# aletheia-labs/qp-zk-circuits-rm

Hardware: AMD Instinct MI355X
Metric: Wormhole proofs/sec (whole node) (higher is better)
Workload: dtype u64 (Goldilocks field); 1 GPU; batch256_wormhole_proofs_per_gpu; circuit=wormhole deg13 (135 wires), batch_per_gpu=256, provers_per_gpu=3, step_schedule=pipelined, parallelism=proofs sharded x1, RCCL gather of leaf proofs

## Files before the change

### include/qpgpu.h

```cpp
#ifndef QPGPU_H
#define QPGPU_H
#include <stddef.h>
#include <stdint.h>

#ifdef __cplusplus
extern "C" {
#endif

typedef enum {
    QP_OK = 0,
    QP_ERR_ARG = 1,
    QP_ERR_HIP = 2,
    QP_ERR_OOM = 3,
    QP_ERR_STATE = 4,
    QP_ERR_WITNESS = 5,
    QP_ERR_FORMAT = 6
} qp_status;

typedef struct qp_ctx qp_ctx;
typedef struct qp_batch qp_batch;

int qp_ctx_create(int device, qp_ctx **out);
void qp_ctx_destroy(qp_ctx *ctx);
const char *qp_ctx_last_error(const qp_ctx *ctx);
// ... 70 lines not shown
int qp_voting_circuit_new(int zero_knowledge, qp_circuit **out);
int qp_voting_commit(const qp_circuit *c, const qp_voting_inputs *in, qp_witness **out, char *err, size_t errcap);
int qp_aggregation_circuit_new(const uint8_t *inner_common, size_t len, uint32_t nproofs, qp_circuit **out);
typedef struct {
    const uint8_t *verifier_only;
    size_t vlen;
    const uint8_t *const *proofs;
    const size_t *lens;
    uint32_t nproofs;
    const uint64_t *zk_randomness;
} qp_aggregation_chunk;
int qp_aggregation_commit(const qp_circuit *c, const uint8_t *verifier_only, size_t vlen,
                          const uint8_t *const *proofs, const size_t *lens, uint32_t nproofs,
                          const uint64_t *zk_randomness, qp_witness **out, char *err, size_t errcap);
int qp_witness_wires(const qp_witness *w, uint64_t *out);
int qp_witness_public_inputs(const qp_witness *w, uint64_t *out, uint32_t cap, uint32_t *n);
void qp_witness_free(qp_witness *w);

typedef struct qp_prover qp_prover;
int qp_prover_new(qp_ctx *ctx, const qp_circuit *c, uint32_t max_batch, qp_prover **out);
void qp_prover_free(qp_prover *p);
int qp_prover_proof_size(const qp_prover *p, size_t *len);
int qp_prover_verifier_data(const qp_prover *p, uint8_t *out, size_t cap, size_t *len);
int qp_prover_prove(qp_prover *p, const qp_witness *const *w, uint32_t nproofs, uint8_t *out, size_t stride,
                    size_t *lens);
int qp_prover_prove_wires(qp_prover *p, const uint64_t *wires, const uint64_t *pis, uint32_t nproofs, uint8_t *out,
                          size_t stride, size_t *lens);
int qp_prover_prove_wormhole_inputs(qp_prover *p, const qp_wormhole_inputs *in, uint32_t nproofs, uint8_t *out,
                                    size_t stride, size_t *lens);
int qp_prover_prove_voting_inputs(qp_prover *p, const qp_voting_inputs *in, uint32_t nproofs, uint8_t *out,
                                  size_t stride, size_t *lens);
int qp_prover_prove_aggregation(qp_prover *p, const qp_aggregation_chunk *chunks, uint32_t nchunks, uint8_t *out,
                                size_t stride, size_t *lens);
int qp_prover_prove_wires_dev(qp_prover *p, const uint64_t *d_wires, const uint64_t *pis, uint32_t nproofs,
                              uint8_t *out, size_t stride, size_t *lens);
int qp_prover_set_timing(qp_prover *p, int enable);
int qp_prover_debug_force_pow(qp_prover *p, uint64_t witness, int enable);
int qp_prover_debug_drop_table(qp_prover *p, const char *name);
enum {
    QP_FOP_NT_ADD = 0,
    QP_FOP_NT_ADD4,
    QP_FOP_GFN_ADD,
    QP_FOP_GFN_ADD_C,
    QP_FOP_PF_ADD_C,
    QP_FOP_GL_ADD,
    QP_FOP_NT_SUB,
    QP_FOP_NT_SUB4,
    QP_FOP_GL_SUB,
    QP_FOP_NT_REDUCE,
    QP_FOP_GFN_REDUCE,
    QP_FOP_GL_REDUCE128,
    QP_FOP_PF_REDUCE_ROW,
    QP_FOP_PF_REDUCE_ROW_C,
    QP_FOP_PF_SUB_SMALL,
    QP_FOP_PF_MUL,
    QP_FOP_PF_MUL_C,
    QP_FOP_PF_MULK2,
    QP_FOP_PF_MULK3,
    QP_FOP_GL_MUL,
    QP_FOP_PF_SBOX,
    QP_FOP_PF_SBOX_C,
    QP_FOP_NT_MUL_POW2,
    QP_FOP_ACC3,
    QP_FOP_COUNT
};
int qp_debug_field_op(qp_ctx *ctx, uint32_t op, uint32_t param, const uint64_t *a, const uint64_t *b, uint64_t n,
                      uint64_t *out);
enum {
    QP_PFORM_PERMUTE_NC = 0,
    QP_PFORM_PERMUTE_CAPZ,
    QP_PFORM_ROUNDS1_L7,
    QP_PFORM_COOP_PERMUTE,
    QP_PFORM_ROW_PERMUTE,
    QP_PFORM_MDS_BLOCK,
    QP_PFORM_MDS_K,
    QP_PFORM_MDS_MADS,
    QP_PFORM_CAPZ_ROUND0,
    QP_PFORM_MDS_INIT_SPARSE,
    QP_PFORM_PARTIAL_GROUP,
    QP_PFORM_FULL_ROUND_DYN,
    QP_PFORM_PARTIAL_DYN,
    QP_PFORM_COOP_MDS,
    QP_PFORM_ROW_MDS,
    QP_PFORM_COUNT
};
int qp_debug_poseidon_op(qp_ctx *ctx, uint32_t form, uint32_t param, const uint64_t *states, uint64_t nstates,
                         uint64_t *out);
int qp_prover_set_host_threads(qp_prover *p, uint32_t nthreads);
int qp_prover_kernel_stats(qp_prover *p, double *ms, double *units, uint64_t *launches, uint32_t n, int reset);
int qp_prover_stage_times(qp_prover *p, double *ms, uint32_t n, int reset);

typedef struct qp_registry qp_registry;
int qp_registry_new(qp_ctx *ctx, const uint64_t *keys, uint64_t n, qp_registry **out);
void qp_registry_free(qp_registry *r);
int qp_registry_root(const qp_registry *r, uint64_t out[4]);
int qp_registry_size(const qp_registry *r, uint64_t *n, uint32_t *max_depth);
int qp_registry_paths(qp_registry *r, const uint64_t *idx, uint32_t nidx, uint64_t *siblings, uint32_t *path_bits,
                      uint32_t *depth);
int qp_registry_level(qp_registry *r, uint32_t level, uint64_t *out, uint64_t *len);
int qp_registry_build_times(const qp_registry *r, double ms[3]);

int qp_registry_new_commitments(qp_ctx *ctx, const uint64_t *leaves, uint64_t n, uint64_t capacity, qp_registry **out);
int qp_registry_append(qp_registry *r, const uint64_t *leaves, uint64_t k, uint64_t *first);
int qp_registry_replace(qp_registry *r, const uint64_t *idx, const uint64_t *leaves, uint32_t k);
int qp_registry_reserve(qp_registry *r, uint64_t new_capacity);
int qp_registry_state(const qp_registry *r, uint64_t *capacity, uint64_t *epoch);
typedef struct {
    uint64_t proposal_id[4];
    uint8_t vote;
    const uint64_t *zk_randomness;
} qp_vote_ballot;
int qp_prover_prove_voters(qp_prover *p, qp_registry *r, const uint64_t *idx, const qp_vote_ballot *ballots,
                           uint32_t nproofs, uint8_t *out, size_t stride, size_t *lens);

typedef enum {
    QP_BALLOT_COUNTED = 0,
    QP_BALLOT_PROOF_REJECTED = 1,
    QP_BALLOT_MALFORMED = 2,
    QP_BALLOT_WRONG_PROPOSAL = 3,
    QP_BALLOT_UNKNOWN_ROOT = 4,
    QP_BALLOT_BAD_VOTE = 5,
    QP_BALLOT_DOUBLE_VOTE = 6
} qp_ballot_status;
typedef struct qp_ballot_box qp_ballot_box;
struct qp_verifier;
typedef struct {
    uint32_t status;
    uint32_t verify_status;
    uint64_t number;
    uint64_t first;
} qp_ballot_result;
int qp_ballot_box_new(qp_ctx *ctx , const uint64_t proposal_id[4], const uint64_t *roots,
                      uint32_t nroots, uint64_t capacity, qp_ballot_box **out);
void qp_ballot_box_free(qp_ballot_box *b);
const char *qp_ballot_box_last_error(const qp_ballot_box *b);
int qp_ballot_box_accept_root(qp_ballot_box *b, const uint64_t root[4]);
int qp_ballot_box_cast(qp_ballot_box *b, struct qp_verifier *v, const uint8_t *const *proofs, const size_t *lens,
                       uint32_t n, qp_ballot_result *out);
int qp_ballot_box_cast_public(qp_ballot_box *b, const uint64_t *pis, const uint32_t *verdicts, uint32_t n,
                              qp_ballot_result *out);
int qp_ballot_box_reserve(qp_ballot_box *b, uint64_t new_capacity);
int qp_ballot_box_tally(const qp_ballot_box *b, uint64_t *yes, uint64_t *no);
int qp_ballot_box_state(const qp_ballot_box *b, uint64_t *cast, uint64_t *admitted, uint64_t *capacity);
int qp_ballot_box_entries(qp_ballot_box *b, uint64_t first, uint64_t k, uint64_t *nullifiers, uint64_t *numbers,
                          uint8_t *flags);
int qp_ballot_box_recount(qp_ballot_box *b, uint64_t out[4]);
int qp_ballot_box_cast_times(const qp_ballot_box *b, double ms[2]);


enum { QP_GATE_NOOP = 0 , QP_GATE_CONSTANT = 1 , QP_GATE_PUBLIC_INPUT = 2 ,
       QP_GATE_BASE_SUM = 3 , QP_GATE_ARITHMETIC = 4 , QP_GATE_POSEIDON = 5 ,
       QP_GATE_ARITHMETIC_EXTENSION = 6 , QP_GATE_MUL_EXTENSION = 7 ,
       QP_GATE_RANDOM_ACCESS = 8 , QP_GATE_EXPONENTIATION = 9 , QP_GATE_REDUCING = 10 ,
       QP_GATE_REDUCING_EXTENSION = 11 , QP_GATE_POSEIDON_MDS = 12 ,
       QP_GATE_COSET_INTERPOLATION = 13  };
#define QP_MAX_GATES 16

typedef struct {
    uint32_t num_gates;
    uint32_t kind[QP_MAX_GATES];
    uint32_t param[QP_MAX_GATES];
    uint32_t param2[QP_MAX_GATES];
    uint32_t param3[QP_MAX_GATES];
    uint32_t selector_index[QP_MAX_GATES];
    uint32_t num_selectors;
    uint32_t group_lo[QP_MAX_GATES], group_hi[QP_MAX_GATES];
// ... 72 lines not shown
```

### qp-zk-circuits-rm_amd/csrc/poseidon_fast.h

```cpp
#pragma once
#include <stdint.h>
#include <hip/hip_runtime.h>
#include "field_nc.h"
#include "poseidon.h"
#include "poseidon_partial_consts.h"

namespace pf {

using gfn::EPS;
using gfn::canon;
using gfn::hi32;
using gfn::lo32;
using gfn::mul;
using gfn::mul_c;

template <int C>
__device__ __forceinline__ uint64_t mad_c(uint32_t x, uint64_t add) {
  uint64_t r, cdummy;
  asm("v_mad_u64_u32 %0, %1, %2, %3, %4" : "=v"(r), "=s"(cdummy) : "v"(x), "i"(C), "v"(add));
  return r;
}
template <int C>
__device__ __forceinline__ uint64_t mad_cs(uint32_t x, uint64_t add) {
  uint64_t r, cdummy;
  asm("v_mad_u64_u32 %0, %1, %2, %3, %4" : "=v"(r), "=s"(cdummy) : "v"(x), "i"(C), "s"(add));
  return r;
}

__device__ __forceinline__ uint64_t reduce_row(uint64_t al, uint64_t ah) {
  uint64_t t, c1, c2;
  uint32_t e;
  asm("v_mad_u64_u32 %0, %1, %2, -1, %3" : "=v"(t), "=s"(c1) : "v"(hi32(ah)), "v"(al));
  uint32_t t0 = lo32(t), t1 = hi32(t);
  asm("v_add_co_u32_e64 %0, %1, %2, %3" : "=v"(t1), "=s"(c2) : "v"(t1), "v"(lo32(ah)));
  asm(QP_CWAIT "v_cndmask_b32_e64 %0, 0, -1, %1" : "=v"(e) : "s"(c2));
  const uint64_t tt = ((uint64_t)t1 << 32) | t0;
  uint64_t r;
  asm("v_mad_u64_u32 %0, %1, %2, 1, %3" : "=v"(r), "=s"(c1) : "v"(e), "v"(tt));
  return r;
}

__device__ __forceinline__ uint64_t reduce_row_c(uint64_t al, uint64_t ah) {
  const uint64_t t = al + (ah >> 32) * EPS;
  const uint32_t t1 = hi32(t) + lo32(ah);
  const uint64_t r = ((uint64_t)t1 << 32) | lo32(t);
  return t1 < lo32(ah) ? r + EPS : r;
}
__device__ __forceinline__ uint64_t sbox_c(uint64_t x) {
  const uint64_t x2 = mul_c(x, x);
  const uint64_t x3 = mul_c(x2, x);
  const uint64_t x4 = mul_c(x2, x2);
  return mul_c(x3, x4);
}

__device__ __forceinline__ uint64_t sbox(uint64_t x) {
  const uint64_t x2 = mul(x, x);
  const uint64_t x3 = mul(x2, x);
  const uint64_t x4 = mul(x2, x2);
  return mul(x3, x4);
}

__device__ __forceinline__ void sbox12(uint64_t s[12]) {
#pragma unroll
  for (int i = 0; i < 12; i++) s[i] = sbox(s[i]);
}

__device__ __forceinline__ uint64_t add_c(uint64_t a, uint64_t c) {
  const uint64_t s = a + c;
  return s + (s < c ? EPS : 0);
}

template <int R, int I>
__device__ __forceinline__ void row_terms(uint64_t &al, uint64_t &ah, const uint32_t lo[12], const uint32_t hi[12]) {
  if constexpr (I < 12) {
    constexpr int C = (int)ps::mds_circ(I) + ((R == 0 && I == 0) ? 8 : 0);
    al = mad_c<C>(lo[(I + R) % 12], al);
    ah = mad_c<C>(hi[(I + R) % 12], ah);
    row_terms<R, I + 1>(al, ah, lo, hi);
  }
}

template <int R>
__device__ __forceinline__ void mds_rows_k(uint64_t s[12], const uint32_t lo[12], const uint32_t hi[12],
                                           const uint64_t k[12]) {
  if constexpr (R < 12) {
    constexpr int C0 = (int)ps::mds_circ(0) + (R == 0 ? 8 : 0);
    uint64_t al = mad_cs<C0>(lo[R], k[R] & EPS);
// ... 199 lines not shown
    const uint32_t v = H ? hi32(s[J]) : lo32(s[J]);
    if constexpr (c != 0) asm("v_mad_u64_u32 %0, vcc, %1, %2, %0" : "+v"(S[K]) : "v"(v), "s"(c) : "vcc");
    if constexpr (K < 2) sparse_row0_h<T, J, H, K + 1>(S, s);
    else if constexpr (H == 0) sparse_row0_h<T, J, 1, 0>(S, s);
    else sparse_row0_h<T, J + 1, 0, 0>(S, s);
  }
}

__device__ __forceinline__ uint64_t sub_small(uint64_t r, uint32_t y0, uint32_t y1) {
  uint32_t r0 = lo32(r), r1 = hi32(r), e;
  uint64_t c;
  asm("v_sub_co_u32_e64 %0, %1, %2, %3" : "=v"(r0), "=s"(c) : "v"(r0), "v"(y0));
  asm(QP_CWAIT "v_subb_co_u32_e64 %0, %1, %2, %3, %4" : "=v"(r1), "=s"(c) : "v"(r1), "v"(y1), "s"(c));
  asm(QP_CWAIT "v_cndmask_b32_e64 %0, 0, -1, %1" : "=v"(e) : "s"(c));
  asm("v_sub_co_u32_e64 %0, %1, %2, %3" : "=v"(r0), "=s"(c) : "v"(r0), "v"(e));
  asm(QP_CWAIT "v_subb_co_u32_e64 %0, %1, %2, 0, %3" : "=v"(r1), "=s"(c) : "v"(r1), "s"(c));
  return ((uint64_t)r1 << 32) | r0;
}

constexpr int PF_GROUP = 4;
struct NoHook {
  __device__ __forceinline__ uint64_t operator()(int, uint64_t v) const { return v; }
};

template <int T0, int M, int L = 0>
__device__ __forceinline__ void group_gammas(uint64_t &al, uint64_t &ah, const uint32_t (*l)[3]) {
  if constexpr (L < M) {
    mac_limbs<PT_GAM, ((T0 + M) * 22 + T0 + L) * 6>(al, ah, l[L]);
    group_gammas<T0, M, L + 1>(al, ah, l);
  }
}

template <int T0, int G, int M = 0, class HK>
__device__ __forceinline__ void group_lane0(const uint64_t s[12], uint64_t &s0, uint32_t (*l)[3], const HK &hook) {
  if constexpr (M < G) {
    constexpr int T = T0 + M;
    const uint64_t x = sbox(hook(T, s0));
    limbs22(x, l[M]);
    constexpr uint32_t kl = pfp::K0[2 * T], kh = pfp::K0[2 * T + 1];
    uint64_t S[3];
    asm("v_mad_u64_u32 %0, vcc, %1, 25, %2" : "=v"(S[0]) : "v"(lo32(x)), "s"((uint64_t)kl) : "vcc");
    S[1] = (uint64_t)hi32(x) * 25600u;
    S[2] = 0;
    sparse_row0_h<T>(S, s);
    uint64_t al = S[0] + (uint64_t)lo32(S[1]) * (1u << 22);
    uint64_t ah = (uint64_t)kh + (uint64_t)hi32(S[1]) * (1u << 22);
    ah += (uint64_t)lo32(S[2]) * (1u << 12);
    ah += (uint64_t)hi32(S[2]) * (1u << 12);
    group_gammas<T0, M>(al, ah, l);
    s0 = sub_small(reduce_row(al, ah), hi32(S[2]) << 12, hi32(S[2]) >> 20);
    group_lane0<T0, G, M + 1>(s, s0, l, hook);
  }
}

template <int T0, int G, int I, int M>
__device__ __forceinline__ void group_col_macs(uint64_t &bl, uint64_t &bh, const uint32_t (*l)[3]) {
  if constexpr (M < G) {
    mac_limbs<PT_BV, ((T0 + M) * 11 + I - 1) * 6>(bl, bh, l[M]);
    group_col_macs<T0, G, I, M + 1>(bl, bh, l);
  }
}

template <int T0, int G, int I = 1>
__device__ __forceinline__ void group_cols(uint64_t s[12], const uint32_t (*l)[3]) {
  if constexpr (I < 12) {
    constexpr bool last = T0 + G == 22;
    uint64_t bl = (uint64_t)lo32(s[I]) + (last ? pfp::KLAST[2 * I] : 0u);
    uint64_t bh = (uint64_t)hi32(s[I]) + (last ? pfp::KLAST[2 * I + 1] : 0u);
    group_col_macs<T0, G, I, 0>(bl, bh, l);
    s[I] = reduce_row(bl, bh);
    group_cols<T0, G, I + 1>(s, l);
  }
}

template <int T0, int G, class HK = NoHook>
__device__ __forceinline__ void partial_group(uint64_t s[12], const HK &hook = HK{}) {
  uint32_t l[G][3];
  uint64_t s0 = s[0];
  group_lane0<T0, G>(s, s0, l, hook);
  group_cols<T0, G>(s, l);
  s[0] = s0;
}

template <int R, uint32_t OUT = 0xFFFu>
__device__ __forceinline__ void rounds(uint64_t s[12]) {
  if constexpr (R == 3) {
    sbox12(s);
    mds_init_sparse(s);
    rounds<4, OUT>(s);
  } else if constexpr (R >= 4 && R < 26) {
    constexpr int T0 = R - 4, G = (22 - T0) < PF_GROUP ? (22 - T0) : PF_GROUP;
    static_assert(G > 1, "22 partial rounds in groups of PF_GROUP leave no single round");
    partial_group<T0, G>(s);
    rounds<R + G, OUT>(s);
  } else if constexpr (R < 30) {
    sbox12(s);
    if constexpr (R == 29) mds_block<-1, OUT>(s);
    else mds_block<R + 1>(s);
    rounds<R + 1, OUT>(s);
  }
}

template <int R, int I = 0>
__device__ __forceinline__ void capz_row_terms(uint64_t &al, uint64_t &ah, const uint32_t lo[12], const uint32_t hi[12]) {
  if constexpr (I < 12) {
    constexpr int J = (I + R) % 12;
    if constexpr (J < 8) {
      constexpr int C = (int)ps::mds_circ(I) + ((R == 0 && I == 0) ? 8 : 0);
      al = mad_c<C>(lo[J], al);
      ah = mad_c<C>(hi[J], ah);
    }
    capz_row_terms<R, I + 1>(al, ah, lo, hi);
  }
}
template <int R = 0>
__device__ __forceinline__ void capz_mds(uint64_t s[12], const uint32_t lo[12], const uint32_t hi[12]) {
  if constexpr (R < 12) {
    uint64_t al = pfp::CAPZ_K[2 * R], ah = pfp::CAPZ_K[2 * R + 1];
    capz_row_terms<R>(al, ah, lo, hi);
    s[R] = reduce_row(al, ah);
    capz_mds<R + 1>(s, lo, hi);
  }
}

template <uint32_t OUT = 0xFFFu>
__device__ __forceinline__ void permute_nc_capz(uint64_t s[12]) {
  uint32_t lo[12], hi[12];
#pragma unroll
  for (int i = 0; i < 8; i++) {
    s[i] = sbox(add_c(s[i], ps::rc_cx(i)));
    lo[i] = lo32(s[i]);
    hi[i] = hi32(s[i]);
  }
  capz_mds(s, lo, hi);
  rounds<1, OUT>(s);
}

__device__ __forceinline__ void permute_nc(uint64_t s[12]) {
#pragma unroll
  for (int i = 0; i < 12; i++) s[i] = add_c(s[i], ps::rc_cx(i));
  rounds<0>(s);
}

__device__ __forceinline__ void permute(uint64_t s[12]) {
  permute_nc(s);
#pragma unroll
  for (int i = 0; i < 12; i++) s[i] = canon(s[i]);
}

}
```

### qp-zk-circuits-rm_amd/csrc/poseidon_probe.hip

```cpp
#include "../../include/qpgpu.h"
#include <algorithm>
#include <string>
#include "ctx.h"
#include "poseidon.h"
#include "poseidon_coop.h"
#include "poseidon_fast.h"

namespace {

constexpr int MDS_NEXT = 27;

bool wave_form(uint32_t f) { return f == QP_PFORM_COOP_PERMUTE || f == QP_PFORM_COOP_MDS; }
bool row_form(uint32_t f) { return f == QP_PFORM_ROW_PERMUTE || f == QP_PFORM_ROW_MDS; }
bool capz_form(uint32_t f) { return f == QP_PFORM_PERMUTE_CAPZ || f == QP_PFORM_CAPZ_ROUND0; }

bool param_ok(uint32_t form, uint32_t param) {
  switch (form) {
    case QP_PFORM_MDS_BLOCK: return param == 0 || param == MDS_NEXT;
    case QP_PFORM_MDS_K:
    case QP_PFORM_FULL_ROUND_DYN:
    case QP_PFORM_PARTIAL_DYN: return param >= 1 && param < (uint32_t)ps::ROUNDS;
    case QP_PFORM_PARTIAL_GROUP: return param <= 20 && param % pf::PF_GROUP == 0;
    default: return form < QP_PFORM_COUNT && !param;
  }
}

__device__ __forceinline__ void split(const uint64_t s[12], uint32_t lo[12], uint32_t hi[12]) {
#pragma unroll
  for (int i = 0; i < 12; i++) {
    lo[i] = pf::lo32(s[i]);
    hi[i] = pf::hi32(s[i]);
  }
}

template <uint32_t FORM, int P>
__global__ void __launch_bounds__(256) k_poseidon_lane(const uint64_t *__restrict__ in, uint64_t nstates,
                                                       uint32_t param, uint64_t *__restrict__ out) {
  for (uint64_t g = (uint64_t)blockIdx.x * blockDim.x + threadIdx.x; g < nstates;
       g += (uint64_t)gridDim.x * blockDim.x) {
    uint64_t s[12];
#pragma unroll
    for (int i = 0; i < 12; i++) s[i] = in[12 * g + i];
    if constexpr (FORM == QP_PFORM_PERMUTE_NC) {
      pf::permute_nc(s);
    } else if constexpr (FORM == QP_PFORM_PERMUTE_CAPZ) {
      pf::permute_nc_capz<0xFu>(s);
    } else if constexpr (FORM == QP_PFORM_ROUNDS1_L7) {
      pf::rounds<1, 0x80u>(s);
    } else if constexpr (FORM == QP_PFORM_MDS_BLOCK) {
      pf::mds_block<P>(s);
    } else if constexpr (FORM == QP_PFORM_MDS_K) {
      uint64_t k[12];
#pragma unroll
      for (int i = 0; i < 12; i++) k[i] = ps::RC_DEV[param * 12 + i];
      pf::mds_k(s, k);
    } else if constexpr (FORM == QP_PFORM_MDS_MADS) {
      pf::mds_mads(s);
    } else if constexpr (FORM == QP_PFORM_CAPZ_ROUND0) {
      uint32_t lo[12], hi[12];
#pragma unroll
      for (int i = 0; i < 8; i++) {
        s[i] = pf::sbox(pf::add_c(s[i], ps::rc_cx(i)));
        lo[i] = pf::lo32(s[i]);
        hi[i] = pf::hi32(s[i]);
      }
      pf::capz_mds(s, lo, hi);
    } else if constexpr (FORM == QP_PFORM_MDS_INIT_SPARSE) {
      pf::mds_init_sparse(s);
    } else if constexpr (FORM == QP_PFORM_PARTIAL_GROUP) {
      pf::partial_group<P, (22 - P) < pf::PF_GROUP ? (22 - P) : pf::PF_GROUP>(s);
    } else if constexpr (FORM == QP_PFORM_FULL_ROUND_DYN) {
      pf::full_round_dyn(s, ps::RC_DEV + param * 12);
    } else {
      static_assert(FORM == QP_PFORM_PARTIAL_DYN, "one-lane form");
      s[0] = pf::sbox(s[0]);
      uint32_t lo[12], hi[12];
      split(s, lo, hi);
      pf::mds_rows_block_dyn<0>(s, lo, hi, ps::RC_DEV + param * 12);
    }
#pragma unroll
    for (int i = 0; i < 12; i++) out[12 * g + i] = s[i];
  }
}

template <uint32_t FORM>
__global__ void __launch_bounds__(256) k_poseidon_coop(const uint64_t *__restrict__ in, uint64_t nstates,
                                                       uint64_t *__restrict__ out) {
  constexpr bool ROW = FORM == QP_PFORM_ROW_PERMUTE || FORM == QP_PFORM_ROW_MDS;
  const uint64_t st = ROW ? (uint64_t)blockIdx.x * 16 + (threadIdx.x >> 4) : (uint64_t)blockIdx.x * 4 + (threadIdx.x >> 6);
  const uint32_t lane = threadIdx.x & (ROW ? 15 : 63);
  if (st >= nstates) return;
  uint64_t x = lane < 12 ? in[12 * st + lane] : 0;
  if constexpr (FORM == QP_PFORM_COOP_PERMUTE) {
    x = pc::permute(x);
  } else if constexpr (FORM == QP_PFORM_ROW_PERMUTE) {
    x = pc::permute_row(x);
  } else {
    uint32_t coef[12];
    pc::mds_coef(lane < 12 ? lane : 0, coef);
    if constexpr (FORM == QP_PFORM_COOP_MDS) x = pc::wave_mds_row(x, coef);
    else x = pc::row_mds(x, coef);
  }
  if (lane < 12) out[12 * st + lane] = x;
}

template <uint32_t FORM, int P>
void lane_launch(dim3 grid, hipStream_t s, const uint64_t *in, uint64_t n, uint32_t param, uint64_t *out) {
  k_poseidon_lane<FORM, P><<<grid, 256, 0, s>>>(in, n, param, out);
}

template <int T0 = 0>
void group_launch(uint32_t t0, dim3 grid, hipStream_t s, const uint64_t *in, uint64_t n, uint64_t *out) {
  if constexpr (T0 < 22) {
    if (t0 == (uint32_t)T0) lane_launch<QP_PFORM_PARTIAL_GROUP, T0>(grid, s, in, n, 0, out);
    else group_launch<T0 + pf::PF_GROUP>(t0, grid, s, in, n, out);
  }
}

void launch(uint32_t form, uint32_t param, hipStream_t s, const uint64_t *in, uint64_t n, uint64_t *out) {
  if (wave_form(form) || row_form(form)) {
    const dim3 grid((unsigned)((n + (row_form(form) ? 15 : 3)) / (row_form(form) ? 16 : 4)));
    switch (form) {
      case QP_PFORM_COOP_PERMUTE: k_poseidon_coop<QP_PFORM_COOP_PERMUTE><<<grid, 256, 0, s>>>(in, n, out); break;
      case QP_PFORM_ROW_PERMUTE: k_poseidon_coop<QP_PFORM_ROW_PERMUTE><<<grid, 256, 0, s>>>(in, n, out); break;
      case QP_PFORM_COOP_MDS: k_poseidon_coop<QP_PFORM_COOP_MDS><<<grid, 256, 0, s>>>(in, n, out); break;
      default: k_poseidon_coop<QP_PFORM_ROW_MDS><<<grid, 256, 0, s>>>(in, n, out); break;
    }
    return;
  }
  const dim3 grid((unsigned)std::min<uint64_t>((n + 255) / 256, 1024));
  switch (form) {
    case QP_PFORM_PERMUTE_NC: lane_launch<QP_PFORM_PERMUTE_NC, 0>(grid, s, in, n, param, out); break;
    case QP_PFORM_PERMUTE_CAPZ: lane_launch<QP_PFORM_PERMUTE_CAPZ, 0>(grid, s, in, n, param, out); break;
    case QP_PFORM_ROUNDS1_L7: lane_launch<QP_PFORM_ROUNDS1_L7, 0>(grid, s, in, n, param, out); break;
    case QP_PFORM_MDS_BLOCK:
      if (param) lane_launch<QP_PFORM_MDS_BLOCK, MDS_NEXT>(grid, s, in, n, param, out);
      else lane_launch<QP_PFORM_MDS_BLOCK, -1>(grid, s, in, n, param, out);
      break;
    case QP_PFORM_MDS_K: lane_launch<QP_PFORM_MDS_K, 0>(grid, s, in, n, param, out); break;
    case QP_PFORM_MDS_MADS: lane_launch<QP_PFORM_MDS_MADS, 0>(grid, s, in, n, param, out); break;
    case QP_PFORM_CAPZ_ROUND0: lane_launch<QP_PFORM_CAPZ_ROUND0, 0>(grid, s, in, n, param, out); break;
    case QP_PFORM_MDS_INIT_SPARSE: lane_launch<QP_PFORM_MDS_INIT_SPARSE, 0>(grid, s, in, n, param, out); break;
    case QP_PFORM_PARTIAL_GROUP: group_launch(param, grid, s, in, n, out); break;
    case QP_PFORM_FULL_ROUND_DYN: lane_launch<QP_PFORM_FULL_ROUND_DYN, 0>(grid, s, in, n, param, out); break;
    default: lane_launch<QP_PFORM_PARTIAL_DYN, 0>(grid, s, in, n, param, out); break;
  }
}

}

extern "C" int qp_debug_poseidon_op(qp_ctx *c, uint32_t form, uint32_t param, const uint64_t *states,
                                    uint64_t nstates, uint64_t *out) {
  if (!c) return QP_ERR_ARG;
  if (!param_ok(form, param)) { c->err = "qp_debug_poseidon_op: unknown form or parameter"; return QP_ERR_ARG; }
  if (nstates > ((uint64_t)1 << 20)) { c->err = "qp_debug_poseidon_op: more than 2^20 states"; return QP_ERR_ARG; }
  if (!nstates) return QP_OK;
  if (!states || !out) { c->err = "null argument"; return QP_ERR_ARG; }
  if (capz_form(form))
    for (uint64_t i = 0; i < nstates; i++)
      if (states[12 * i + 8] | states[12 * i + 9] | states[12 * i + 10] | states[12 * i + 11]) {
        c->err = "qp_debug_poseidon_op: lanes 8..11 of a capz state must be 0";
        return QP_ERR_ARG;
      }
  const uint64_t n = nstates * 12;
  DevBuf din, dout;
  hipError_t e = hipSetDevice(c->device);
  if (!e) e = din.alloc(n);
  if (!e) e = dout.alloc(n);
  if (!e) e = hipMemcpyAsync(din.p, states, n * 8, hipMemcpyHostToDevice, c->stream);
  if (!e) {
    launch(form, param, c->stream, din.p, nstates, dout.p);
    e = hipGetLastError();
  }
  if (!e) e = hipMemcpyAsync(out, dout.p, n * 8, hipMemcpyDeviceToHost, c->stream);
  if (!e) e = hipStreamSynchronize(c->stream);
  if (e) {
    c->err = std::string("qp_debug_poseidon_op: ") + hipGetErrorString(e);
    return e == hipErrorOutOfMemory ? QP_ERR_OOM : QP_ERR_HIP;
  }
  return QP_OK;
}
```

### qp-zk-circuits-rm_amd/qp_wormhole/_native.py

```python
import ctypes
import os
import re

import numpy as np

HERE = os.path.dirname(os.path.abspath(__file__))
LIB_PATH = os.environ.get("QPGPU_LIB") or os.path.join(HERE, "libqpgpu.so")
HEADER = os.path.join(os.path.dirname(os.path.dirname(HERE)), "include", "qpgpu.h")

U64P = np.ctypeslib.ndpointer(np.uint64, flags="C_CONTIGUOUS")
U32P = np.ctypeslib.ndpointer(np.uint32, flags="C_CONTIGUOUS")
U8P = np.ctypeslib.ndpointer(np.uint8, flags="C_CONTIGUOUS")
VP = ctypes.c_void_p
PP = ctypes.POINTER(ctypes.c_void_p)

STATUS = {0: "QP_OK", 1: "QP_ERR_ARG", 2: "QP_ERR_HIP", 3: "QP_ERR_OOM", 4: "QP_ERR_STATE",
          5: "QP_ERR_WITNESS", 6: "QP_ERR_FORMAT"}


MAX_GATES = 16
GATE_KINDS = ["noop", "constant", "public_input", "base_sum", "arithmetic", "poseidon", "arithmetic_extension",
              "mul_extension", "random_access", "exponentiation", "reducing", "reducing_extension", "poseidon_mds",
              "coset_interpolation"]

# ... 250 lines not shown
        rc = lib().qp_commit_coeffs(ctx.h, coeffs, npolys, log_n, rate_bits, cap_height,
                                    None if salt_c is None else salt_c.ctypes.data, nsalt, cap,
                                    ctypes.byref(h) if keep else None)
        ctx.check(rc, "qp_commit_coeffs")
        return cls(ctx, h if keep else None, npolys, nsalt, log_n, rate_bits, cap_height, cap, coeffs)

    def open(self, indices):
        idx = np.ascontiguousarray(indices, dtype=np.uint32)
        W = self.npolys + self.nsalt
        depth = self.log_n + self.rate_bits - self.cap_height
        leaves = np.zeros((len(idx), W), np.uint64)
        sibs = np.zeros((len(idx), depth, 4), np.uint64)
        self.ctx.check(lib().qp_batch_open(self.h, idx, len(idx), leaves, sibs), "qp_batch_open")
        return leaves, sibs

    def eval_ext(self, points, first=0, npolys=None):
        pts = _ext_points(points)
        npolys = self.npolys - first if npolys is None else npolys
        if first < 0 or npolys < 1 or first + npolys > self.npolys:
            raise ValueError(f"window [{first}, {first + npolys}) outside the batch's {self.npolys} polynomials")
        out = np.zeros((pts.shape[0], npolys, 2), np.uint64)
        self.ctx.check(lib().qp_batch_eval_ext(self.h, first, npolys, pts, pts.shape[0], out), "qp_batch_eval_ext")
        return out

    def lde(self):
        out = np.zeros((self.npolys, 1 << (self.log_n + self.rate_bits)), np.uint64)
        self.ctx.check(lib().qp_batch_lde(self.h, out), "qp_batch_lde")
        return out

    def free(self):
        if self.h:
            lib().qp_batch_free(self.h)
            self.h = None

    def __del__(self):
        try:
            self.free()
        except Exception:
            pass


def ifft(ctx, data):
    a = np.ascontiguousarray(data, dtype=np.uint64).copy()
    ncols, n = a.shape
    ctx.check(lib().qp_ifft(ctx.h, a, ncols, n.bit_length() - 1), "qp_ifft")
    return a


def lde(ctx, coeffs, rate_bits, shift=0xC65C18B67785D900):
    c = np.ascontiguousarray(coeffs, dtype=np.uint64)
    ncols, n = c.shape
    out = np.zeros((ncols, n << rate_bits), np.uint64)
    ctx.check(lib().qp_lde(ctx.h, c, ncols, n.bit_length() - 1, rate_bits, shift, out), "qp_lde")
    return out


def poseidon_permute(ctx, states):
    s = np.ascontiguousarray(states, dtype=np.uint64).copy()
    ctx.check(lib().qp_poseidon_permute(ctx.h, s, s.shape[0]), "qp_poseidon_permute")
    return s


(FOP_NT_ADD, FOP_NT_ADD4, FOP_GFN_ADD, FOP_GFN_ADD_C, FOP_PF_ADD_C, FOP_GL_ADD, FOP_NT_SUB, FOP_NT_SUB4, FOP_GL_SUB,
 FOP_NT_REDUCE, FOP_GFN_REDUCE, FOP_GL_REDUCE128, FOP_PF_REDUCE_ROW, FOP_PF_REDUCE_ROW_C, FOP_PF_SUB_SMALL,
 FOP_PF_MUL, FOP_PF_MUL_C, FOP_PF_MULK2, FOP_PF_MULK3, FOP_GL_MUL, FOP_PF_SBOX, FOP_PF_SBOX_C, FOP_NT_MUL_POW2,
 FOP_ACC3, FOP_COUNT) = range(25)


def debug_field_op(ctx, op, a, b=None, param=0):
    a = np.ascontiguousarray(a, dtype=np.uint64).ravel()
    if b is not None:
        b = np.ascontiguousarray(b, dtype=np.uint64).ravel()
        if b.size != a.size:
            raise ValueError("a and b differ in length")
    nout = a.size // param if op == FOP_ACC3 and param and a.size % param == 0 else a.size
    out = np.zeros(nout, np.uint64)
    ctx.check(lib().qp_debug_field_op(ctx.h, int(op), int(param), a, None if b is None else b.ctypes.data, a.size,
                                      out), "qp_debug_field_op")
    return out


(PFORM_PERMUTE_NC, PFORM_PERMUTE_CAPZ, PFORM_ROUNDS1_L7, PFORM_COOP_PERMUTE, PFORM_ROW_PERMUTE, PFORM_MDS_BLOCK,
 PFORM_MDS_K, PFORM_MDS_MADS, PFORM_CAPZ_ROUND0, PFORM_MDS_INIT_SPARSE, PFORM_PARTIAL_GROUP, PFORM_FULL_ROUND_DYN,
 PFORM_PARTIAL_DYN, PFORM_COOP_MDS, PFORM_ROW_MDS, PFORM_COUNT) = range(16)


def debug_poseidon_op(ctx, form, states, param=0):
    if states is None:
        n, src = 1, None
    else:
        s = np.ascontiguousarray(states, dtype=np.uint64).reshape(-1, 12)
        n, src = s.shape[0], s.ctypes.data
    out = np.zeros((n, 12), np.uint64)
    ctx.check(lib().qp_debug_poseidon_op(ctx.h, int(form), int(param), src, n, out.ctypes.data),
              "qp_debug_poseidon_op")
    return out


def hash_no_pad(values):
    a = np.ascontiguousarray(values, dtype=np.uint64)
    out = np.zeros(4, np.uint64)
    rc = lib().qp_hash_no_pad(a, len(a), out)
    if rc:
        raise QpError(rc, "qp_hash_no_pad")
    return [int(x) for x in out]



def gate_desc(circuit):
    g = GateDesc()
    rc = lib().qp_circuit_gate_desc(circuit.h, ctypes.byref(g))
    if rc:
        raise QpError(rc, "qp_circuit_gate_desc")
    return g


def _u64(v, n=None):
    a = np.ascontiguousarray([int(x) for x in v] if not isinstance(v, np.ndarray) else v, dtype=np.uint64)
    if n is not None and a.size != n:
        raise ValueError(f"expected {n} values, got {a.size}")
    return a


def quotient(ctx, cs, wires, zs_pp, gd, betas, gammas, alphas, pi_hash):
    nc, qdf = gd.num_challenges, gd.quotient_degree_factor
    out = np.zeros((nc * qdf, 1 << cs.log_n), np.uint64)
    ctx.check(lib().qp_quotient(ctx.h, cs.h, wires.h, zs_pp.h, ctypes.byref(gd), _u64(betas, nc), _u64(gammas, nc),
                                _u64(alphas, nc), _u64(pi_hash, 4), out), "qp_quotient")
    return out


class FriLayer:

    def __init__(self, ctx, coeffs, log_values, shift, arity_bits, cap_height):
        c = np.ascontiguousarray(coeffs, dtype=np.uint64)
        if c.ndim != 2 or c.shape[0] != 2:
            raise ValueError("coeffs must be [2][2^k] (ext c0 row, c1 row)")
        self.ctx, self.log_values, self.arity_bits, self.cap_height = ctx, log_values, arity_bits, cap_height
        self.cap = np.zeros((1 << cap_height, 4), np.uint64)
        h = ctypes.c_void_p()
        ctx.check(lib().qp_fri_layer_commit(ctx.h, c, c.shape[1].bit_length() - 1, log_values, shift, arity_bits,
                                            cap_height, self.cap, ctypes.byref(h)), "qp_fri_layer_commit")
        self.h = h

    def open(self, indices):
        idx = np.ascontiguousarray(indices, dtype=np.uint32)
        depth = self.log_values - self.arity_bits - self.cap_height
        evals = np.zeros((len(idx), 1 << self.arity_bits, 2), np.uint64)
        sibs = np.zeros((len(idx), depth, 4), np.uint64)
        self.ctx.check(lib().qp_fri_layer_open(self.h, idx, len(idx), evals, sibs), "qp_fri_layer_open")
        return evals, sibs

    def free(self):
        if self.h:
            lib().qp_fri_layer_free(self.h)
            self.h = None

    def __del__(self):
        try:
            self.free()
        except Exception:
            pass


def fri_fold(ctx, coeffs, arity_bits, beta):
    c = np.ascontiguousarray(coeffs, dtype=np.uint64)
    out = np.zeros((2, c.shape[1] >> arity_bits), np.uint64)
# ... 84 lines not shown
```

Before: 1227 proofs/s.

## Evaluate Poseidon partial rounds as dense grouped small-integer matrix products

Replaces the sparse-matrix partial-round path (mds_init_sparse followed by partial_group) with dense_group. Each group of up to three partial rounds is evaluated with precomputed powers of the MDS matrix, whose entries are small integers, plus folded round constants. Every output row is a chain of 32-bit multiply-adds on the lo/hi limbs with one reduction at the end, so there are fewer reductions and no sparse-matrix change of basis. The cost is more multiply-adds per group, and constants that do not fit as inline immediates go through SGPRs. A debug probe form is added to test the new group function.

```diff
diff --git a/include/qpgpu.h b/include/qpgpu.h
--- a/include/qpgpu.h
+++ b/include/qpgpu.h
@@ -176,6 +176,7 @@
     QP_PFORM_PARTIAL_DYN,
     QP_PFORM_COOP_MDS,
     QP_PFORM_ROW_MDS,
+    QP_PFORM_DENSE_GROUP,
     QP_PFORM_COUNT
 };
 int qp_debug_poseidon_op(qp_ctx *ctx, uint32_t form, uint32_t param, const uint64_t *states, uint64_t nstates,
diff --git a/qp-zk-circuits-rm_amd/csrc/poseidon_dense_consts.h b/qp-zk-circuits-rm_amd/csrc/poseidon_dense_consts.h
--- /dev/null
+++ b/qp-zk-circuits-rm_amd/csrc/poseidon_dense_consts.h
@@ -0,0 +1,116 @@
+#pragma once
+#include <stdint.h>
+namespace pfd {
+constexpr int GLEN[22] = {3, 0, 0, 3, 0, 0, 3, 0, 0, 3, 0, 0, 3, 0, 0, 3, 0, 0, 2, 0, 2, 0};
+constexpr uint32_t POW[396] = {
+    15u, 41u, 16u, 2u, 28u, 13u, 13u, 39u, 18u, 34u, 20u,
+    17u, 15u, 41u, 16u, 2u, 28u, 13u, 13u, 39u, 18u, 34u,
+    20u, 17u, 15u, 41u, 16u, 2u, 28u, 13u, 13u, 39u, 18u,
+    34u, 20u, 17u, 15u, 41u, 16u, 2u, 28u, 13u, 13u, 39u,
+    18u, 34u, 20u, 17u, 15u, 41u, 16u, 2u, 28u, 13u, 13u,
+    39u, 18u, 34u, 20u, 17u, 15u, 41u, 16u, 2u, 28u, 13u,
+    13u, 39u, 18u, 34u, 20u, 17u, 15u, 41u, 16u, 2u, 28u,
+    13u, 13u, 39u, 18u, 34u, 20u, 17u, 15u, 41u, 16u, 2u,
+    28u, 13u, 13u, 39u, 18u, 34u, 20u, 17u, 15u, 41u, 16u,
+    2u, 28u, 13u, 13u, 39u, 18u, 34u, 20u, 17u, 15u, 41u,
+    16u, 2u, 28u, 13u, 13u, 39u, 18u, 34u, 20u, 17u, 15u,
+    41u, 16u, 2u, 28u, 13u, 13u, 39u, 18u, 34u, 20u, 17u,
+    5577u, 3889u, 4968u, 6188u, 4656u, 4977u, 5755u, 4895u, 4430u, 5968u, 4864u,
+    5006u, 5012u, 4266u, 5200u, 5662u, 4872u, 4938u, 5196u, 5198u, 4056u, 6146u,
+    4694u, 3912u, 5288u, 4518u, 4288u, 5780u, 4690u, 3872u, 5364u, 4402u, 4056u,
+    6276u, 4466u, 5018u, 5796u, 4082u, 5006u, 5988u, 4430u, 4874u, 5364u, 5198u,
+    4151u, 4947u, 4580u, 5228u, 4740u, 4079u, 4733u, 4701u, 4430u, 3872u, 5196u,
+    5363u, 4203u, 6338u, 5178u, 4942u, 5663u, 4417u, 4733u, 5988u, 4690u, 4938u,
+    5781u, 5025u, 4528u, 6520u, 4840u, 5137u, 5663u, 4079u, 5006u, 5780u, 4872u,
+    4778u, 4828u, 5110u, 4680u, 5762u, 4840u, 4942u, 4740u, 4082u, 4288u, 5662u,
+    5102u, 5116u, 5944u, 5554u, 4680u, 6520u, 5178u, 5228u, 5796u, 4518u, 5200u,
+    5982u, 4476u, 4942u, 5944u, 5110u, 4528u, 6338u, 4580u, 5018u, 5288u, 4266u,
+    4625u, 4541u, 4476u, 5116u, 4828u, 5025u, 4203u, 4947u, 4466u, 3912u, 5012u,
+    4361u, 4625u, 5982u, 5102u, 4778u, 5781u, 5363u, 4151u, 6276u, 4694u, 5006u,
+    1214817u, 1089681u, 1265600u, 1256596u, 1145944u, 1308833u, 1199363u, 1101695u, 1264278u, 1095368u, 1177368u,
+    1245100u, 1098072u, 1190716u, 1300784u, 1133572u, 1206472u, 1279668u, 1065320u, 1209572u, 1138800u, 1175868u,
+    1078368u, 1034088u, 1115568u, 1149856u, 1093360u, 1118088u, 1092896u, 1040696u, 1097728u, 966368u, 1138800u,
+    1205802u, 1101998u, 1269500u, 1268360u, 1156924u, 1283798u, 1207246u, 1100850u, 1297432u, 1097728u, 1209572u,
+    1134223u, 997679u, 1083496u, 1182252u, 1052008u, 1106983u, 1138253u, 964737u, 1100850u, 1040696u, 1065320u,
+    1229703u, 1139523u, 1217028u, 1273780u, 1206844u, 1246827u, 1220837u, 1138253u, 1207246u, 1092896u, 1279668u,
+    1215705u, 1128169u, 1287344u, 1286388u, 1160104u, 1302425u, 1246827u, 1106983u, 1283798u, 1118088u, 1206472u,
+    1229284u, 1046872u, 1170628u, 1251568u, 1103164u, 1160104u, 1206844u, 1052008u, 1156924u, 1093360u, 1133572u,
+    1269180u, 1199540u, 1256688u, 1367024u, 1251568u, 1286388u, 1273780u, 1182252u, 1268360u, 1149856u, 1300784u,
+    1204572u, 1096600u, 1299092u, 1256688u, 1170628u, 1287344u, 1217028u, 1083496u, 1269500u, 1115568u, 1190716u,
+    1137505u, 1024929u, 1096600u, 1199540u, 1046872u, 1128169u, 1139523u, 997679u, 1101998u, 1034088u, 1098072u,
+    1202205u, 1137505u, 1204572u, 1269180u, 1229284u, 1215705u, 1229703u, 1134223u, 1205802u, 1078368u, 1245100u,
+};
+constexpr uint32_t COL[36] = {
+    25u, 20u, 34u, 18u, 39u, 13u, 13u, 28u, 2u, 16u, 41u, 15u,
+    5017u, 4864u, 5968u, 4430u, 4895u, 5755u, 4977u, 4656u, 6188u, 4968u, 3889u, 5577u,
+    1259209u, 1177368u, 1095368u, 1264278u, 1101695u, 1199363u, 1308833u, 1145944u, 1256596u, 1265600u, 1089681u, 1214817u,
+};
+constexpr uint32_t K[528] = {
+    0x268d7d8cu, 0x7131aa45u, 0x95630f9fu, 0x93510360u, 0xafc26bfbu, 0xad535b24u, 0x993e44beu, 0x4627f5c6u,
+    0xb8f1cc58u, 0x645cf794u, 0x0af61617u, 0x241c70edu, 0x647905f1u, 0xacb8e076u, 0x4c4f474du, 0x3737e9dbu,
+    0xe75fffb6u, 0xe7ea5e33u, 0xc9bfc23au, 0x90dee49fu, 0x6bc09c92u, 0xd1b1edf7u, 0xa645c602u, 0x0b65481bu,
+    0xde0778d0u, 0xf1417c86u, 0x3e3a4221u, 0xcb1e1ea5u, 0xa1cc7354u, 0x70ef5db2u, 0x8153cebdu, 0x8cf2fe12u,
+    0x0bb238d1u, 0x0cde9575u, 0x23fda7ddu, 0xa8ec9318u, 0x649fc4dcu, 0x216e7231u, 0x5c2dfa6bu, 0x2b1acc12u,
+    0x7a497c60u, 0xc986e6fau, 0xe9f52f30u, 0x15c97929u, 0x5c51b9d5u, 0x9882c5c7u, 0x12c450abu, 0x0dbe3cd9u,
+    0x1ef1f717u, 0xbe56ca78u, 0xa029077bu, 0x9a8644b3u, 0x268817e7u, 0x52b02192u, 0x582f33a3u, 0x0abc5297u,
+    0x7990679au, 0xe54f22eeu, 0xa2518f18u, 0xa469d6aeu, 0x37b273ccu, 0xbb1b667du, 0xa2a4519du, 0x3c358ffbu,
+    0x410f63fau, 0xbe01b370u, 0x8b5714f8u, 0xd5ba62f7u, 0xd89243c8u, 0x20bf71b9u, 0x70c921f3u, 0x7af4c52bu,
+    0xc3ac118eu, 0x7159cd30u, 0xafead540u, 0x839b4e8fu, 0x82920adcu, 0x0d3f3e5eu, 0xdee7bba8u, 0x8f7d83bdu,
+    0xea071d06u, 0x780f2243u, 0xf3de1634u, 0xeb915845u, 0x26b6f386u, 0xd19e120du, 0x7e5fecc6u, 0x016ee53au,
+    0x7933e477u, 0xcb5fd54eu, 0x79fd449fu, 0xacb84178u, 0xe7f74732u, 0x9c22190bu, 0xa3ba3621u, 0x5d693c1bu,
+    0x6ff4f0e2u, 0x3efc7580u, 0xdd2c3a4au, 0x1ad28a69u, 0xa19bc3eau, 0xa6d4683cu, 0xe4c0c964u, 0x58f93708u,
+    0x24eccac6u, 0x5c04e8bbu, 0x77b734e2u, 0xa0ddb923u, 0x2acf8837u, 0x51b1c235u, 0x90ec02fbu, 0xa3a7540du,
+    0x7dfd0efdu, 0x044f27afu, 0xbb81e245u, 0xc46f260cu, 0xc0c9fa66u, 0x2fc0ad68u, 0x78581623u, 0x5048239au,
+    0xfd0a553bu, 0x854e26e7u, 0xa714d050u, 0x6e2d494du, 0xb9653dfdu, 0x15536d53u, 0x3f2ac720u, 0xdc1b3579u,
+    0xd71b5368u, 0x371b585eu, 0x3e2320abu, 0x4ca149f2u, 0x0194e8f8u, 0x7c4fd5dau, 0xa5ac26e0u, 0x44d6d6eau,
+    0xe6151b8fu, 0x6e4712cfu, 0xe0558d8au, 0x44680366u, 0x6da2cab4u, 0x0839ba7cu, 0xe2327e99u, 0x586a9fb8u,
+    0x93258387u, 0x30a46805u, 0x61bd9ce1u, 0x337dc00cu, 0xc7a4ff1du, 0xd5eca244u, 0x64d279bdu, 0x77626382u,
+    0xdeefd767u, 0xc1e434beu, 0x53b8ec22u, 0x0299351au, 0xad251b80u, 0xb2d456e4u, 0xa49cea0bu, 0x3e9ed1fdu,
+    0xa450bed8u, 0x2972a92bu, 0x7be493deu, 0x20216dd7u, 0x28449ec6u, 0xadffe8cfu, 0x4c27d243u, 0x1c4dbb1cu,
+    0x9b604341u, 0xc750352du, 0xe2510474u, 0x2a7eb209u, 0xf36a831fu, 0x0e6eb6d7u, 0x0b22a127u, 0x6b9b88b6u,
+    0x2c25c1e6u, 0xff47920eu, 0x68592caeu, 0x0833b7c1u, 0xe77eb0ffu, 0x1881f3dcu, 0x4eb2e7aau, 0xbf33e669u,
+    0x71ef8563u, 0x1b8a66abu, 0x5ea2333fu, 0x31514bb6u, 0x0198c7f0u, 0xeaf9a168u, 0x0c3f34bdu, 0x4fe8e83cu,
+    0x66e3abc2u, 0xd6b93cc9u, 0x52289282u, 0x36ee51b4u, 0x458f7d4du, 0x1bb20c3au, 0xac80cdfau, 0x1ffdfb49u,
+    0x298022d5u, 0x0fa800e4u, 0xb996bbc1u, 0xdbf976a1u, 0x76f2d4d5u, 0x225b39a1u, 0x69082198u, 0xa45d5e6bu,
+    0xfa675720u, 0x3809a401u, 0xb5c50370u, 0xc2e6704cu, 0x65fbbcd7u, 0x1d5e6b28u, 0x4bb5e49fu, 0x46333421u,
+    0x2d74d7f7u, 0x77500598u, 0xdde6c8b0u, 0x86ab99b4u, 0x3f51c080u, 0xb1204f60u, 0x70250ecfu, 0xef61ac84u,
+    0x132c603fu, 0x1bbcd90fu, 0x964db557u, 0x0cd1dabdu, 0xeb9d1ec9u, 0x11a3ae5bu, 0xa585d11du, 0xf755bfeeu,
+    0x268ea4d7u, 0xa3b83250u, 0x927c93afu, 0x516306f4u, 0xc9efa1dau, 0xddb4ac49u, 0x369d4418u, 0x64bb6decu,
+    0x8a73b798u, 0x3fe3eee0u, 0x0da999fdu, 0xb27e6849u, 0xba0fe83bu, 0xfb25ab8fu, 0x3c9ce9f3u, 0xeb8b25beu,
+    0x9ec6bdafu, 0x0522549cu, 0x4dc0a544u, 0x90a47131u, 0xd8b91f3fu, 0xa23bd396u, 0x0915ac04u, 0x7ae2a33fu,
+    0xbc3b163au, 0x743b355du, 0xabbce758u, 0x376c6631u, 0x067d91f7u, 0x9f4d8482u, 0xcbefe493u, 0xa4779291u,
+    0xd77d2177u, 0x66809a1bu, 0x6b7b1a7bu, 0x25bd84ceu, 0x3047b692u, 0xde59fdeau, 0x10178af1u, 0x75fb00ddu,
+    0x2d9c33ceu, 0x46556f5cu, 0xbd25de10u, 0x699471c4u, 0x632059cbu, 0x2a6ebf09u, 0x8b8c3be9u, 0xa17b5803u,
+    0x82537744u, 0x8fc747beu, 0x429da700u, 0x790d302du, 0xfdf0055eu, 0x2c41991au, 0xc6bfc0abu, 0x32f3edefu,
+    0x00c17442u, 0xdd611f10u, 0xdfea4fd0u, 0xd8185f9au, 0xa9a3ab1eu, 0xef87139cu, 0xc34ee133u, 0x3ba71336u,
+    0x56b70238u, 0x7d3a455du, 0x30182684u, 0x660d32e1u, 0x48cd1f43u, 0x297a863fu, 0xa751ebb7u, 0x90e0a736u,
+    0x550c4fd3u, 0x549f80ceu, 0x2f38bd64u, 0x0f73b292u, 0xfb7a9c3fu, 0x16bf1f73u, 0x005bec17u, 0x6d1f5a59u,
+    0xfac93576u, 0xe44c4dd5u, 0x3b2bd1b2u, 0xf8f7e333u, 0x323037aeu, 0xa0163b05u, 0xf4470f4du, 0xbf4ca328u,
+    0x8b8e9a00u, 0xd921a411u, 0xfe5258ebu, 0x27e3249cu, 0x6d15c097u, 0xfde2a1cfu, 0x79d9678eu, 0x0ac0af72u,
+    0xc095c779u, 0x9f3cf4e5u, 0xee3c1564u, 0x2e0e9083u, 0x7fa411bbu, 0x9289a92cu, 0x77027cd8u, 0x0f73cfc2u,
+    0xd41b033fu, 0x15f154a2u, 0x29688609u, 0xd1795c6eu, 0x116c6ec1u, 0xf3267319u, 0xad93b9ccu, 0x74ee383cu,
+    0xfcd44819u, 0xca17dcb4u, 0x36869a7eu, 0x28eb017cu, 0xc49a303du, 0xd8c39810u, 0xf4f8d367u, 0x91a5e951u,
+    0x8c856749u, 0xb14f64deu, 0xc32305f1u, 0x0e0f4582u, 0x86f7685au, 0x5def8c2eu, 0xc28f9600u, 0x166054a2u,
+    0xd5d01d33u, 0xe89cd854u, 0x8bb882a2u, 0x5cd377dcu, 0x83eee860u, 0xa7b0fb78u, 0xc392950du, 0x7684403eu,
+    0x4fed3b52u, 0x5fa3f06fu, 0x1bc04831u, 0x8df57ac1u, 0x1e1e1897u, 0x2db01efau, 0xaadb9ca2u, 0x54846de4u,
+    0x5893c784u, 0xba674538u, 0x44d2c75bu, 0x541d4963u, 0x74e687feu, 0xe9096784u, 0xf6c9c2ffu, 0xdfe89923u,
+    0x988250a0u, 0x44e8d81au, 0x533eef9au, 0x1ffad092u, 0xd83ca96fu, 0x9ee8a0f6u, 0x31731243u, 0x1b7c46bau,
+    0xfdbb075au, 0x293fe4c4u, 0xdd6421a8u, 0x43e3a80fu, 0x78f532a1u, 0x73283bebu, 0x91b65e3fu, 0x2b464eeeu,
+    0x6c5b695fu, 0x7ff1958cu, 0x68b16dc6u, 0xcda23fbcu, 0x8e38c9b9u, 0x0f20eeadu, 0xca101142u, 0x0dd0c875u,
+    0x53a3e603u, 0x6fa19061u, 0x14b1b0f2u, 0x2f293617u, 0x86303ee1u, 0xfcb08855u, 0xe4dde9b3u, 0x2e17c5d7u,
+    0x53fe1c65u, 0x58d33908u, 0x47d8dcedu, 0xaebfdda0u, 0xe5747ec6u, 0x675d6c7au, 0xd25def23u, 0x27732879u,
+    0x5ccc86e5u, 0xb8d35c9du, 0x081bafe9u, 0x4fe2afbeu, 0xd78e7686u, 0xfd1e3e36u, 0xf66def9cu, 0xb18169e4u,
+    0xe9a39368u, 0xde122bebu, 0x8f002526u, 0x4d001fd5u, 0x0eb4a9f8u, 0xca663700u, 0x24f91f78u, 0x2f2339d6u,
+    0xc80df518u, 0x6d1a7918u, 0x342308e9u, 0xdf9a4939u, 0xe6c8398cu, 0xebc2151eu, 0xa1116515u, 0x03cc2ba8u,
+    0xe840cf83u, 0xd341d037u, 0x5af4afccu, 0x387cb5d2u, 0x22909e87u, 0xbba2515fu, 0x05f38e47u, 0x7248fe77u,
+    0x5d2e95d9u, 0xa7529fb8u, 0x09220173u, 0xebb9a574u, 0x6e81062eu, 0x7e09244cu, 0xc0436f36u, 0x12961d13u,
+    0x4aaa08e7u, 0xfdc791b7u, 0x099ccd48u, 0xcfd1ca57u, 0x1c6f1649u, 0x096cb583u, 0x4f1c9f28u, 0x731bb56au,
+    0xc2a40de8u, 0xd546b0e4u, 0x798241d9u, 0xbe2350d4u, 0x708b0753u, 0x8e1f04cbu, 0xdb2e7a31u, 0x1537ede4u,
+    0xdbbf9facu, 0x1478d361u, 0xd141875cu, 0x6f02dc07u, 0xd8e556a2u, 0x296a202eu, 0x9bf32ee5u, 0x2afd6799u,
+    0xfa95491du, 0x7acfd96eu, 0x0abb2c6du, 0x6798ba0cu, 0x26c92122u, 0x34c6f57bu, 0xd206b5deu, 0x5736e1bau,
+    0x0056521bu, 0x20057d2au, 0xd0578bd7u, 0x3dea5bd5u, 0x7d4634acu, 0x16e50d89u, 0xb9b7a6e3u, 0x29bff3ecu,
+    0xb62c5246u, 0x0950b3ffu, 0x3a062fa0u, 0xadf244e5u, 0x6458edfdu, 0x3d53248bu, 0xe6a555e2u, 0xda74e741u,
+    0xbc8ee641u, 0xfdd5931fu, 0x5a797889u, 0x2f03a5c0u, 0xdae1b4b7u, 0xcd1ca6bdu, 0x80172046u, 0x0b6d590bu,
+    0x4d8d2226u, 0x666db593u, 0x589c3507u, 0xe20f065fu, 0xd6043f99u, 0xa7a632f9u, 0x783f7861u, 0x26582bd3u,
+};
+}
diff --git a/qp-zk-circuits-rm_amd/csrc/poseidon_fast.h b/qp-zk-circuits-rm_amd/csrc/poseidon_fast.h
--- a/qp-zk-circuits-rm_amd/csrc/poseidon_fast.h
+++ b/qp-zk-circuits-rm_amd/csrc/poseidon_fast.h
@@ -3,6 +3,7 @@
 #include <hip/hip_runtime.h>
 #include "field_nc.h"
 #include "poseidon.h"
+#include "poseidon_dense_consts.h"
 #include "poseidon_partial_consts.h"
 
 namespace pf {
@@ -368,16 +369,86 @@
   s[0] = s0;
 }
 
+
+template <uint32_t C>
+__device__ __forceinline__ void mac_pair(uint64_t &al, uint64_t &ah, uint32_t lo, uint32_t hi) {
+  static_assert(C != 0, "the integer rows have no zero entry");
+  if constexpr (C <= 64)
+    asm("v_mad_u64_u32 %0, vcc, %2, %4, %0\n\tv_mad_u64_u32 %1, vcc, %3, %4, %1"
+        : "+v"(al), "+v"(ah) : "v"(lo), "v"(hi), "i"(C) : "vcc");
+  else
+    asm("v_mad_u64_u32 %0, vcc, %2, %4, %0\n\tv_mad_u64_u32 %1, vcc, %3, %4, %1"
+        : "+v"(al), "+v"(ah) : "v"(lo), "v"(hi), "s"(C) : "vcc");
+}
+
+template <int M, int I, int J = 1>
+__device__ __forceinline__ void dg_lane_terms(uint64_t &al, uint64_t &ah, const uint32_t lo[12], const uint32_t hi[12]) {
+  if constexpr (J < 12) {
+    mac_pair<pfd::POW[((M - 1) * 12 + I) * 11 + J - 1]>(al, ah, lo[J], hi[J]);
+    dg_lane_terms<M, I, J + 1>(al, ah, lo, hi);
+  }
+}
+template <int M, int I, int L>
+__device__ __forceinline__ void dg_x_terms(uint64_t &al, uint64_t &ah, const uint32_t *xl, const uint32_t *xh) {
+  if constexpr (L >= 0) {
+    mac_pair<pfd::COL[(M - 1 - L) * 12 + I]>(al, ah, xl[L], xh[L]);
+    dg_x_terms<M, I, L - 1>(al, ah, xl, xh);
+  }
+}
+template <int T0, int M, int I>
+__device__ __forceinline__ uint64_t dg_row(const uint32_t lo[12], const uint32_t hi[12], const uint32_t *xl,
+                                           const uint32_t *xh) {
+  constexpr uint32_t C0 = pfd::COL[I];
+  static_assert(C0 <= 64, "M's column 0 is inline");
+  constexpr uint64_t kl = pfd::K[((T0 + M - 1) * 12 + I) * 2], kh = pfd::K[((T0 + M - 1) * 12 + I) * 2 + 1];
+  uint64_t al, ah;
+  asm("v_mad_u64_u32 %0, vcc, %2, %4, %5\n\tv_mad_u64_u32 %1, vcc, %3, %4, %6"
+      : "=&v"(al), "=&v"(ah) : "v"(xl[M - 1]), "v"(xh[M - 1]), "i"(C0), "s"(kl), "s"(kh) : "vcc");
+  dg_x_terms<M, I, M - 2>(al, ah, xl, xh);
+  dg_lane_terms<M, I>(al, ah, lo, hi);
+  return reduce_row(al, ah);
+}
+
+template <int T0, int G, int M = 1>
+__device__ __forceinline__ void dg_lane0(const uint32_t lo[12], const uint32_t hi[12], uint32_t *xl, uint32_t *xh) {
+  if constexpr (M < G) {
+    const uint64_t x = sbox(dg_row<T0, M, 0>(lo, hi, xl, xh));
+    xl[M] = lo32(x);
+    xh[M] = hi32(x);
+    dg_lane0<T0, G, M + 1>(lo, hi, xl, xh);
+  }
+}
+template <int T0, int G, int I = 0>
+__device__ __forceinline__ void dg_out(uint64_t s[12], const uint32_t lo[12], const uint32_t hi[12], const uint32_t *xl,
+                                       const uint32_t *xh) {
+  if constexpr (I < 12) {
+    s[I] = dg_row<T0, G, I>(lo, hi, xl, xh);
+    dg_out<T0, G, I + 1>(s, lo, hi, xl, xh);
+  }
+}
+
+template <int T0, int G>
+__device__ __forceinline__ void dense_group(uint64_t s[12]) {
+  static_assert(G >= 1 && G <= 3 && T0 >= 0 && T0 + G <= 22, "the tables hold (MZ)^1..3");
+  uint32_t lo[12], hi[12], xl[G], xh[G];
+#pragma unroll
+  for (int j = 1; j < 12; j++) {
+    lo[j] = lo32(s[j]);
+    hi[j] = hi32(s[j]);
+  }
+  const uint64_t x0 = sbox(s[0]);
+  xl[0] = lo32(x0);
+  xh[0] = hi32(x0);
+  dg_lane0<T0, G>(lo, hi, xl, xh);
+  dg_out<T0, G>(s, lo, hi, xl, xh);
+}
+
 template <int R, uint32_t OUT = 0xFFFu>
 __device__ __forceinline__ void rounds(uint64_t s[12]) {
-  if constexpr (R == 3) {
-    sbox12(s);
-    mds_init_sparse(s);
-    rounds<4, OUT>(s);
-  } else if constexpr (R >= 4 && R < 26) {
-    constexpr int T0 = R - 4, G = (22 - T0) < PF_GROUP ? (22 - T0) : PF_GROUP;
-    static_assert(G > 1, "22 partial rounds in groups of PF_GROUP leave no single round");
-    partial_group<T0, G>(s);
+  if constexpr (R >= 4 && R < 26) {
+    constexpr int T0 = R - 4, G = pfd::GLEN[T0];
+    static_assert(G > 0, "partial rounds are entered at a group start");
+    dense_group<T0, G>(s);
     rounds<R + G, OUT>(s);
   } else if constexpr (R < 30) {
     sbox12(s);
diff --git a/qp-zk-circuits-rm_amd/csrc/poseidon_probe.hip b/qp-zk-circuits-rm_amd/csrc/poseidon_probe.hip
--- a/qp-zk-circuits-rm_amd/csrc/poseidon_probe.hip
+++ b/qp-zk-circuits-rm_amd/csrc/poseidon_probe.hip
@@ -21,6 +21,7 @@
     case QP_PFORM_FULL_ROUND_DYN:
     case QP_PFORM_PARTIAL_DYN: return param >= 1 && param < (uint32_t)ps::ROUNDS;
     case QP_PFORM_PARTIAL_GROUP: return param <= 20 && param % pf::PF_GROUP == 0;
+    case QP_PFORM_DENSE_GROUP: return param < 22 && pfd::GLEN[param] != 0;
     default: return form < QP_PFORM_COUNT && !param;
   }
 }
@@ -69,6 +70,8 @@
       pf::mds_init_sparse(s);
     } else if constexpr (FORM == QP_PFORM_PARTIAL_GROUP) {
       pf::partial_group<P, (22 - P) < pf::PF_GROUP ? (22 - P) : pf::PF_GROUP>(s);
+    } else if constexpr (FORM == QP_PFORM_DENSE_GROUP) {
+      pf::dense_group<P, pfd::GLEN[P]>(s);
     } else if constexpr (FORM == QP_PFORM_FULL_ROUND_DYN) {
       pf::full_round_dyn(s, ps::RC_DEV + param * 12);
     } else {
@@ -117,6 +120,14 @@
   }
 }
 
+template <int T0 = 0>
+void dense_launch(uint32_t t0, dim3 grid, hipStream_t s, const uint64_t *in, uint64_t n, uint64_t *out) {
+  if constexpr (T0 < 22) {
+    if (t0 == (uint32_t)T0) lane_launch<QP_PFORM_DENSE_GROUP, T0>(grid, s, in, n, 0, out);
+    else dense_launch<T0 + pfd::GLEN[T0]>(t0, grid, s, in, n, out);
+  }
+}
+
 void launch(uint32_t form, uint32_t param, hipStream_t s, const uint64_t *in, uint64_t n, uint64_t *out) {
   if (wave_form(form) || row_form(form)) {
     const dim3 grid((unsigned)((n + (row_form(form) ? 15 : 3)) / (row_form(form) ? 16 : 4)));
@@ -142,6 +153,7 @@
     case QP_PFORM_CAPZ_ROUND0: lane_launch<QP_PFORM_CAPZ_ROUND0, 0>(grid, s, in, n, param, out); break;
     case QP_PFORM_MDS_INIT_SPARSE: lane_launch<QP_PFORM_MDS_INIT_SPARSE, 0>(grid, s, in, n, param, out); break;
     case QP_PFORM_PARTIAL_GROUP: group_launch(param, grid, s, in, n, out); break;
+    case QP_PFORM_DENSE_GROUP: dense_launch(param, grid, s, in, n, out); break;
     case QP_PFORM_FULL_ROUND_DYN: lane_launch<QP_PFORM_FULL_ROUND_DYN, 0>(grid, s, in, n, param, out); break;
     default: lane_launch<QP_PFORM_PARTIAL_DYN, 0>(grid, s, in, n, param, out); break;
   }
diff --git a/qp-zk-circuits-rm_amd/qp_wormhole/_native.py b/qp-zk-circuits-rm_amd/qp_wormhole/_native.py
--- a/qp-zk-circuits-rm_amd/qp_wormhole/_native.py
+++ b/qp-zk-circuits-rm_amd/qp_wormhole/_native.py
@@ -356,7 +356,7 @@
 
 (PFORM_PERMUTE_NC, PFORM_PERMUTE_CAPZ, PFORM_ROUNDS1_L7, PFORM_COOP_PERMUTE, PFORM_ROW_PERMUTE, PFORM_MDS_BLOCK,
  PFORM_MDS_K, PFORM_MDS_MADS, PFORM_CAPZ_ROUND0, PFORM_MDS_INIT_SPARSE, PFORM_PARTIAL_GROUP, PFORM_FULL_ROUND_DYN,
- PFORM_PARTIAL_DYN, PFORM_COOP_MDS, PFORM_ROW_MDS, PFORM_COUNT) = range(16)
+ PFORM_PARTIAL_DYN, PFORM_COOP_MDS, PFORM_ROW_MDS, PFORM_DENSE_GROUP, PFORM_COUNT) = range(17)
 
 
 def debug_poseidon_op(ctx, form, states, param=0):
```

Measured after the change: 1321 proofs/s (median of 6 runs). 7.7% higher.
